# muzishen/IMAGDressing

Hardware: AMD Instinct MI355X
Metric: 512x512 50-step images/sec (whole node) (higher is better)
Workload: dtype bf16

## Files before the change

imagdressing_amd/_lib.py:

```python
from __future__ import annotations

import ctypes as C
import os

_HERE = os.path.dirname(os.path.abspath(__file__))
LIB_PATH = os.environ.get("IMD_LIB_PATH") or os.path.join(_HERE, "libimagdressing_hip.so")

ABI_VERSION = 9

u16p = C.POINTER(C.c_uint16)
f32p = C.POINTER(C.c_float)


class _Sized(C.Structure):

    def __init__(self, *args, **kw):
        super().__init__(*args, **kw)
        self.struct_bytes = C.sizeof(self)


class HeadsDest(C.Structure):
    _fields_ = [("ptr", C.c_void_p), ("kind", C.c_int), ("DP", C.c_int), ("L", C.c_int), ("scale", C.c_float)]


# ... 1 lines not shown
    _fields_ = [("struct_bytes", C.c_uint32), 
        ("x", C.c_void_p), ("w", C.c_void_p), ("out", C.c_void_p),
        ("M", C.c_int), ("N", C.c_int), ("K", C.c_int),
        ("Cin", C.c_int), ("taps", C.c_int), ("Hin", C.c_int), ("Win", C.c_int), ("Hout", C.c_int),
        ("Wout", C.c_int), ("stride", C.c_int), ("ups", C.c_int),
        ("x_pix_stride", C.c_int), ("out_ld", C.c_int), ("res_ld", C.c_int),
        ("bias", C.c_void_p), ("rowvec", C.c_void_p), ("rowvec_stride", C.c_int),
        ("res", C.c_void_p), ("out_scale", C.c_float), ("act", C.c_int), ("out_f32", C.c_int),
        ("mode", C.c_int), ("hC", C.c_int), ("hH", C.c_int), ("hD", C.c_int),
        ("hd", HeadsDest * 3), ("dtype", C.c_int), ("split_k", C.c_int), ("splitk_ws", C.c_void_p),
        ("x_bytes", C.c_uint32), ("w_bytes", C.c_uint32), ("flags", C.c_int),
        ("gn_a", C.c_void_p), ("gn_b", C.c_void_p), ("gn_silu", C.c_int), ("pad_br_only", C.c_int),
        ("splitk_counters", C.c_void_p),
        ("gn_stats_out", C.c_void_p), ("gn_stats_groups", C.c_int),
        ("gn_in_partial", C.c_void_p), ("gn_in_gamma", C.c_void_p), ("gn_in_beta", C.c_void_p),
        ("gn_in_nparts", C.c_int), ("gn_in_groups", C.c_int), ("gn_in_silu", C.c_int), ("gn_in_eps", C.c_float),
        ("gn_out_gamma", C.c_void_p), ("gn_out_beta", C.c_void_p), ("gn_out_eps", C.c_float), ("gn_out_silu", C.c_int), ("gn_out_groups", C.c_int), ("res_rows", C.c_int),
    ]


class FfParams(_Sized):
    _fields_ = [("struct_bytes", C.c_uint32), ("x", C.c_void_p), ("w1", C.c_void_p), ("b1", C.c_void_p), ("w2", C.c_void_p), ("b2", C.c_void_p), ("out", C.c_void_p),
                ("M", C.c_int), ("C", C.c_int), ("inner", C.c_int), ("x_ld", C.c_int), ("out_ld", C.c_int), ("ln", C.c_int),
                ("ln_eps", C.c_float), ("dtype", C.c_int)]


class AttnParams(_Sized):
    _fields_ = [("struct_bytes", C.c_uint32), 
        ("q", C.c_void_p), ("k1", C.c_void_p), ("v1t", C.c_void_p), ("k2", C.c_void_p), ("v2t", C.c_void_p),
        ("scale2", C.c_void_p), ("out", C.c_void_p),
        ("B", C.c_int), ("H", C.c_int), ("N", C.c_int), ("D", C.c_int),
        ("L1", C.c_int), ("L1P", C.c_int), ("kv1_bdiv", C.c_int),
        ("L2", C.c_int), ("L2P", C.c_int), ("kv2_bdiv", C.c_int),
        ("out_ld", C.c_int), ("dtype", C.c_int), ("flags", C.c_int), ("causal", C.c_int), ("k_pad_one", C.c_int),
        ("proj_w", C.c_void_p), ("proj_b", C.c_void_p), ("proj_res", C.c_void_p), ("proj_out", C.c_void_p),
        ("proj_res_ld", C.c_int), ("proj_out_ld", C.c_int), ("proj_counters", C.c_void_p),
        ("out_dup", C.c_void_p), ("phase2_out", C.c_void_p), ("phase2_rows", C.c_int),
    ]


class GroupNormParams(_Sized):
    _fields_ = [("struct_bytes", C.c_uint32), 
        ("x", C.c_void_p), ("y", C.c_void_p), ("gamma", C.c_void_p), ("beta", C.c_void_p), ("partial", C.c_void_p),
        ("B", C.c_int), ("HW", C.c_int), ("C", C.c_int), ("G", C.c_int), ("x_ld", C.c_int), ("y_ld", C.c_int),
        ("eps", C.c_float), ("silu", C.c_int), ("dtype", C.c_int), ("nparts", C.c_int),
    ]
# ... 28 lines not shown
    "imd_attention": (C.c_int, [C.POINTER(AttnParams), C.c_void_p]),
    "imd_attention_dup_supported": (C.c_int, [C.c_int, C.c_int, C.c_int]),
    "imd_attention_phase_split_supported": (C.c_int, [C.c_int]),
    "imd_attention_fp8": (C.c_int, [C.POINTER(AttnParams), C.c_int, C.c_int, C.c_int, C.c_void_p]),
    "imd_attn_quantize_fp8": (C.c_int, [C.c_void_p, C.c_void_p, C.c_int, C.c_long, C.c_int, C.c_int, C.c_float, C.c_int, C.c_void_p]),
    "imd_set_tuning": (C.c_int, [C.c_int, C.c_int]),
    "imd_get_tuning": (C.c_int, [C.c_int]),
    "imd_attn_padded_dims": (C.c_int, [C.c_int, C.POINTER(C.c_int), C.POINTER(C.c_int)]),
    "imd_groupnorm": (C.c_int, [C.POINTER(GroupNormParams), C.c_void_p]),
    "imd_groupnorm_coeffs": (C.c_int, [C.POINTER(GroupNormParams), C.c_void_p, C.c_void_p, C.c_void_p]),
    "imd_conv_patch_supported": (C.c_int, [C.POINTER(ConvGemmParams)]),
    "imd_conv_patch2_supported": (C.c_int, [C.POINTER(ConvGemmParams)]),
    "imd_conv_patch3_supported": (C.c_int, [C.POINTER(ConvGemmParams)]),
    "imd_conv_patch4_supported": (C.c_int, [C.POINTER(ConvGemmParams)]),
    "imd_conv_img_supported": (C.c_int, [C.POINTER(ConvGemmParams)]),
    "imd_conv_patch_stats_parts": (C.c_int, [C.POINTER(ConvGemmParams)]),
    "imd_conv_gemm_stats_parts": (C.c_int, [C.POINTER(ConvGemmParams), C.c_int]),
    "imd_conv_gemm_gn_out_supported": (C.c_int, [C.POINTER(ConvGemmParams)]),
    "imd_row_linear_gn_in_supported": (C.c_int, [C.POINTER(ConvGemmParams), C.c_int]),
    "imd_gemm_dma_supported": (C.c_int, [C.POINTER(ConvGemmParams)]),
    "imd_row_linear": (C.c_int, [C.POINTER(ConvGemmParams), C.c_int, C.c_float, C.c_void_p]),
    "imd_row_linear_supported": (C.c_int, [C.POINTER(ConvGemmParams)]),
    "imd_ff_geglu": (C.c_int, [C.POINTER(FfParams), C.c_void_p]),
    "imd_groupnorm_workspace_floats": (C.c_int, [C.c_int, C.c_int, C.c_int, C.c_int]),
    "imd_layernorm": (C.c_int, [C.POINTER(LayerNormParams), C.c_void_p]),
    "imd_softmax_rows": (C.c_int, [C.c_void_p, C.c_int, C.c_void_p, C.c_int, C.c_int, C.c_int, C.c_int, C.c_void_p]),
    "imd_ddim_cfg_step": (C.c_int, [C.POINTER(DdimParams), C.c_void_p]),
    "imd_ddim_cfg_step_rows": (C.c_int, [C.POINTER(DdimParams), C.c_void_p, C.c_void_p]),
    "imd_timestep_embedding": (C.c_int, [C.c_void_p, C.c_void_p, C.c_int, C.c_int, C.c_void_p]),
    "imd_add": (C.c_int, [C.c_void_p, C.c_int, C.c_void_p, C.c_int, C.c_void_p, C.c_int, C.c_long, C.c_int, C.c_float, C.c_int, C.c_void_p]),
    "imd_embed_tokens": (C.c_int, [C.c_void_p, C.c_int, C.c_void_p, C.c_int, C.c_void_p, C.c_void_p, C.c_long, C.c_int, C.c_int, C.c_void_p]),
    "imd_vit_assemble": (C.c_int, [C.c_void_p, C.c_void_p, C.c_void_p, C.c_void_p, C.c_int, C.c_int, C.c_int, C.c_int, C.c_void_p]),
    "imd_lincomb": (C.c_int, [C.POINTER(C.c_void_p), C.POINTER(C.c_float), C.c_int, C.c_void_p, C.c_long, C.c_void_p]),
    "imd_copy2d": (C.c_int, [C.c_void_p, C.c_int, C.c_void_p, C.c_int, C.c_long, C.c_int, C.c_void_p]),
    "imd_concat2": (C.c_int, [C.c_void_p, C.c_int, C.c_void_p, C.c_int, C.c_void_p, C.c_void_p, C.c_long, C.c_long, C.c_int, C.c_void_p]),
    "imd_concat2_gn_stats": (C.c_int, [C.c_void_p, C.c_int, C.c_void_p, C.c_int, C.c_void_p, C.c_void_p, C.c_int, C.c_int, C.c_int, C.c_int,
                                       C.c_void_p, C.c_int, C.c_void_p]),
    "imd_groupnorm_parts": (C.c_int, [C.c_int, C.c_int, C.c_int]),
    "imd_f32_to_16": (C.c_int, [C.c_void_p, C.c_void_p, C.c_long, C.c_int, C.c_void_p]),
}

_lib = None


class ImdError(RuntimeError):
    pass
# ... 23 lines not shown
```

imagdressing_amd/adapter/attention_processor.py:

```python
from __future__ import annotations

import math
from typing import Dict, Optional, Tuple

import torch
import torch.nn as nn

from .. import ops

bf16 = torch.bfloat16
LOG2E = math.log2(math.e)


class LoRALinearLayer(nn.Module):

    def __init__(self, in_features, out_features, rank=4, network_alpha=None):
        super().__init__()
        self.down = nn.Linear(in_features, rank, bias=False)
        self.up = nn.Linear(rank, out_features, bias=False)
        self.network_alpha = network_alpha
        self.rank = rank
        nn.init.normal_(self.down.weight, std=1 / rank)
        nn.init.zeros_(self.up.weight)

# ... 61 lines not shown
    if ent is None or ent[0] != key or not all(a is b for a, b in zip(ent[1], srcs)):
        t = torch.cat([t.detach().to(device=device, dtype=want) for t in srcs], 0).contiguous()
        ent = cache[which] = (key, tuple(srcs), t)
    return ent[2]


def _ln_folded_q(attn, gamma: torch.Tensor, beta: torch.Tensor, dtype, device, which: str = "q"):
    mods = [getattr(attn, n) for n in _W_PARTS[which]]
    srcs = tuple(m.weight for m in mods) + (gamma, beta)
    cache = attn.__dict__.setdefault("_imd_wcache", {})
    key = (_version_key(*srcs), dtype, str(device))
    ent = cache.get(which + "_ln")
    if ent is None or ent[0] != key or not all(a is b for a, b in zip(ent[1], srcs)):
        w = torch.cat([m.weight.detach().to(device=device, dtype=dtype) for m in mods], 0)
        ent = cache[which + "_ln"] = (key, srcs, ops.fold_layernorm_affine(w, None, gamma.to(device), beta.to(device)))
    return ent[2]


def _qkv_ln_ok(x: torch.Tensor) -> bool:
    return x.shape[-1] == 320 and x.shape[1] % 128 == 0 and ops.FUSED_LN


FUSED_LN_CHANNELS = (320, 640, 1280)


def _as_tokens(hidden_states: torch.Tensor, dtype):
    shape4 = None
    if hidden_states.dim() == 4:
        b, c, h, w = hidden_states.shape
        shape4 = (b, c, h, w)
        hidden_states = hidden_states.view(b, c, h * w).transpose(1, 2)
    if not hidden_states.is_cuda:
        from .._lib import ImdError
        raise ImdError("imagdressing_amd processors run on MI355X only: hidden_states is on " + str(hidden_states.device))
    return hidden_states.to(dtype).contiguous(), shape4


def _restore(out, shape4, like):
    if shape4 is not None:
        b, c, h, w = shape4
        out = out.transpose(-1, -2).reshape(b, c, h, w)
    return out


def _project_kv(tokens: torch.Tensor, wkv: torch.Tensor, heads: int):
    Bk, Lk, Kd = tokens.shape
# ... 93 lines not shown
        Be = ehs.shape[0]
        if B % Be:
            raise ValueError(f"encoder_hidden_states batch {Be} does not divide hidden_states batch {B}")
        return B // Be

    @staticmethod
    def _finish(attn, out, residual_given, like, shape4, ln_fused=False):
        if getattr(attn, "residual_connection", False) and not residual_given:
            if ln_fused:
                raise NotImplementedError("attn.residual_connection together with the engine's fused LayerNorm (imd_layernorm)")
            out = ops.add(out, _as_tokens(like, out.dtype)[0])
        if getattr(attn, "rescale_output_factor", 1.0) != 1.0:
            raise NotImplementedError("rescale_output_factor != 1 is not used by SD1.5")
        out = _restore(out, shape4, like)
        return out if out.dtype == like.dtype else out.to(like.dtype)


class AttnProcessor2_0(_FusedBase):

    fused_layernorm = True

    def __init__(self, cache_entries: int = 256):
        self._text = _TensorCache(capacity=cache_entries)

    def __call__(self, attn, hidden_states, encoder_hidden_states=None, attention_mask=None, temb=None, scale=1.0,
                 imd_residual=None, imd_layernorm=None, **kwargs):
        dt = _compute_dtype(attn, hidden_states, attention_mask)
        x, shape4 = _as_tokens(hidden_states, dt)
        dev = x.device
        wo, bo = _layer_weights(attn, "o", dt, dev), _layer_weights(attn, "bo", dt, dev)
        q_ln = None
        if imd_layernorm is not None:
            g, be, eps = imd_layernorm
            if encoder_hidden_states is not None and x.shape[-1] in FUSED_LN_CHANNELS:
                q_ln = _ln_folded_q(attn, g, be, dt, dev) + (eps,)
            elif encoder_hidden_states is None and _qkv_ln_ok(x):
                q_ln = _ln_folded_q(attn, g, be, dt, dev, "qkv") + (eps,)
            else:
                x = ops.layer_norm(x, g, be, eps)
        if encoder_hidden_states is None:
            out = _fused_attention(x, attn.heads, wq_or_qkv=_layer_weights(attn, "qkv", dt, dev), self_attn=True, wo=wo, bo=bo,
                                   residual=imd_residual, q_ln=q_ln)
        else:
            srcs = (encoder_hidden_states, attn.to_k.weight, attn.to_v.weight)
            kv = self._text.get(srcs, extra=(dt,))
            if kv is None:
                e = encoder_hidden_states.to(device=dev, dtype=dt).contiguous()
                kv = self._text.put(srcs, _project_kv(e, _layer_weights(attn, "kv", dt, dev), attn.heads), extra=(dt,))
            out = _fused_attention(x, attn.heads, wq_or_qkv=_layer_weights(attn, "q", dt, dev), self_attn=False, kv1=kv,
                                   kv1_bdiv=self._ehs_bdiv(x.shape[0], encoder_hidden_states), wo=wo, bo=bo,
                                   residual=imd_residual, q_ln=q_ln)
        return self._finish(attn, out, imd_residual is not None, hidden_states, shape4, ln_fused=imd_layernorm is not None)
# ... 339 lines not shown
```

imagdressing_amd/csrc/capi.cpp:

```cpp
#include <atomic>
#include <mutex>
#include <stdarg.h>
#include <stdio.h>
#include <string.h>

#include "imd_kernels.h"

namespace {
thread_local char g_err[512] = "";
}

int imd_set_error(const char* fmt, ...) {
    va_list ap;
    va_start(ap, fmt);
    vsnprintf(g_err, sizeof(g_err), fmt, ap);
    va_end(ap);
    return 1;
}

int imd_check_launch(const char* what) {
    hipError_t e = hipGetLastError();
    if (e != hipSuccess) return imd_set_error("%s: launch failed: %s", what, hipGetErrorString(e));
    return 0;
}
// ... 178 lines not shown
    if (p->mode == IMD_OUT_HEADS) {
        IMD_REQUIRE(p->hC > 0 && p->hH > 0 && p->hD > 0 && p->hC == p->hH * p->hD && p->N % p->hC == 0 && p->N / p->hC <= 3 && p->hD % 8 == 0,
                    "row_linear: bad head split C=%d H=%d D=%d", p->hC, p->hH, p->hD);
        IMD_REQUIRE(!p->out_f32, "row_linear: head-split output excludes fp32 output");
    }
    IMD_REQUIRE(!ln || ln_eps > 0.f, "row_linear: LayerNorm needs eps > 0");
    if (p->K == 320 && p->N == 960 && p->mode == IMD_OUT_HEADS) {
        IMD_REQUIRE(p->gn_in_partial == nullptr, "row_linear: the fused q / k / v projection has no GroupNorm prologue (gn_in_*)");
        return imd_launch_row_qkv(*p, ln, ln_eps, (hipStream_t)stream);
    }
    if (p->K == 640) return imd_launch_row_linear_k640(*p, ln, ln_eps, (hipStream_t)stream);
    if (p->K == 1280) return imd_launch_row_linear_k1280(*p, ln, ln_eps, (hipStream_t)stream);
    return imd_launch_row_linear(*p, ln, ln_eps, (hipStream_t)stream);
}

int imd_ff_geglu(const imd_ff_params* p, void* stream) {
    IMD_REQUIRE(p != nullptr, "ff_geglu: null params");
    IMD_REQUIRE_SIZE(p, "ff_geglu");
    IMD_REQUIRE(p->x && p->w1 && p->b1 && p->w2 && p->b2 && p->out, "ff_geglu: null pointer");
    IMD_REQUIRE(!p->ln || p->ln_eps > 0.f, "ff_geglu: LayerNorm needs eps > 0");
    return imd_launch_ff_geglu(*p, (hipStream_t)stream);
}

int imd_layernorm(const imd_layernorm_params* p, void* stream) {
    IMD_REQUIRE(p != nullptr, "layernorm: null params");
    IMD_REQUIRE_SIZE(p, "layernorm");
    IMD_REQUIRE(p->x && p->y && p->gamma && p->beta, "layernorm: null pointer");
    return imd_launch_layernorm(*p, (hipStream_t)stream);
}

int imd_embed_tokens(const uint16_t* table, int vocab, const uint16_t* pos, int T, const int64_t* ids, uint16_t* out, long rows, int C,
                     int dtype, void* stream) {
    IMD_REQUIRE(table && pos && ids && out, "embed_tokens: null pointer");
    return imd_launch_embed_tokens(table, vocab, pos, T, ids, out, rows, C, dtype, (hipStream_t)stream);
}

int imd_vit_assemble(const uint16_t* patches, const uint16_t* cls, const uint16_t* pos, uint16_t* out, int B, int P, int C, int dtype,
                     void* stream) {
    IMD_REQUIRE(patches && cls && pos && out, "vit_assemble: null pointer");
    return imd_launch_vit_assemble(patches, cls, pos, out, B, P, C, dtype, (hipStream_t)stream);
}

int imd_lincomb(const float* const* xs, const float* coefs, int n, float* out, long numel, void* stream) {
    IMD_REQUIRE(xs && coefs && out, "lincomb: null pointer");
    return imd_launch_lincomb(xs, coefs, n, out, numel, (hipStream_t)stream);
}
// ... 57 lines not shown
```

imagdressing_amd/csrc/imd_kernels.h:

```cpp
#pragma once
#include <hip/hip_runtime.h>
#include <stdint.h>

#include "../../include/imagdressing_hip.h"

typedef uint16_t bf16_t;
typedef imd_heads_dest HeadsDest;
typedef imd_conv_gemm_params ConvGemmParams;
typedef imd_attn_params AttnParams;
typedef imd_groupnorm_params GroupNormParams;
typedef imd_layernorm_params LayerNormParams;
typedef imd_ddim_params DdimParams;

enum { ACT_NONE = IMD_ACT_NONE, ACT_SILU = IMD_ACT_SILU, ACT_GEGLU = IMD_ACT_GEGLU, ACT_GELU = IMD_ACT_GELU, ACT_QUICK_GELU = IMD_ACT_QUICK_GELU };
enum { OUT_ROWMAJOR = IMD_OUT_ROWMAJOR, OUT_HEADS = IMD_OUT_HEADS };

int imd_set_error(const char* fmt, ...);
int imd_check_launch(const char* what);
int imd_lds_attr(const void* kern, int bytes, const char* what);
int imd_cu_count8();

int imd_conv_gemm_choose_cfg(int M, int N);
int imd_conv_gemm_choose_split(int M, int N, int K, int cfg);
int imd_launch_conv_gemm(const ConvGemmParams& p, int cfg, hipStream_t s);
// ... 9 lines not shown
bool imd_conv_patch64_supported(const ConvGemmParams& p);
int imd_launch_conv_patch64(const ConvGemmParams& p, hipStream_t s);
bool imd_conv_img_supported(const ConvGemmParams& p);
int imd_launch_conv_img(const ConvGemmParams& p, hipStream_t s);
int imd_conv_patch_stats_parts_of(const ConvGemmParams& p);
int imd_conv_gemm_stats_parts_of(const ConvGemmParams& p, int cfg);
bool imd_conv_gemm_gn_out_supported_of(const ConvGemmParams& p, int cfg);
bool imd_row_linear_gn_in_supported_of(const ConvGemmParams& p, int cfg);
int imd_launch_conv_patch(const ConvGemmParams& p, hipStream_t s);
bool imd_row_linear_supported(const ConvGemmParams& p);
int imd_launch_row_linear(const ConvGemmParams& p, int ln, float ln_eps, hipStream_t s);
bool imd_row_linear_k640_supported(const ConvGemmParams& p);
int imd_launch_row_linear_k640(const ConvGemmParams& p, int ln, float ln_eps, hipStream_t s);
bool imd_row_linear_k1280_supported(const ConvGemmParams& p);
int imd_launch_row_linear_k1280(const ConvGemmParams& p, int ln, float ln_eps, hipStream_t s);
bool imd_row_qkv_supported(const ConvGemmParams& p);
int imd_launch_row_qkv(const ConvGemmParams& p, int ln, float ln_eps, hipStream_t s);
bool imd_gemm_dma_supported(const ConvGemmParams& p);
int imd_launch_gemm_dma(const ConvGemmParams& p, hipStream_t s);
int imd_launch_gemm_dma128(const ConvGemmParams& p, int stages, hipStream_t s);
int imd_launch_gemm_dma256(const ConvGemmParams& p, int form, hipStream_t s);
bool imd_conv_dma_supported(const ConvGemmParams& p);
int imd_launch_ff_geglu(const imd_ff_params& p, hipStream_t s);
int imd_launch_attention(const AttnParams& p, hipStream_t s);
int imd_launch_attention_d40(const AttnParams& p, int variant, hipStream_t s);
int imd_launch_attention_fp8(const AttnParams& p, int eq, int ek, int ev, hipStream_t s);
int imd_launch_attn_quantize_fp8(const bf16_t* src, unsigned char* dst, int kind, long rows_or_groups, int LP, int exp2_scale,
                                 float pad_val, int dtype, hipStream_t s);
extern int g_attn_qw40;
extern int g_attn_xcd;
#ifdef IMD_ATTN_SWEEP
extern int g_attn_v80, g_attn_v160;
#endif
extern int g_gemm_flags;
int imd_attn_dpk(int D);
int imd_attn_dpv(int D);
int imd_launch_groupnorm(const GroupNormParams& p, hipStream_t s);
int imd_launch_groupnorm_coeffs(const GroupNormParams& p, float* ca, float* cb, hipStream_t s);
int imd_groupnorm_parts_of(int B, int HW, int C);
int imd_launch_concat2_gn_stats(const bf16_t* a, int Ca, const bf16_t* b, int Cb, const bf16_t* b_add, bf16_t* out, int B, int HW, int b_B, int G,
                                float* partial, int dtype, hipStream_t s);
int imd_launch_layernorm(const LayerNormParams& p, hipStream_t s);
int imd_launch_softmax_rows(const float* s_in, int s_ld, bf16_t* p_out, int p_ld, int rows, int cols, int dtype, hipStream_t s);
int imd_launch_ddim_cfg_step(const DdimParams& p, hipStream_t s);
int imd_launch_ddim_cfg_step_rows(const DdimParams& p, const float* guidance, hipStream_t s);
int imd_launch_timestep_embedding(const float* t, float* out, int B, int dim, hipStream_t s);
// ... 8 lines not shown
```

imagdressing_amd/ops.py:

```python
from __future__ import annotations

import functools
import ctypes as C
from typing import Dict, Optional, Sequence, Tuple

import torch

from . import _lib as L

ACT_NONE, ACT_SILU, ACT_GEGLU, ACT_GELU, ACT_QUICK_GELU = 0, 1, 2, 3, 4
bf16 = torch.bfloat16
f16 = torch.float16
DTYPE_CODE = {torch.bfloat16: 0, torch.float16: 1}


def _code(t: torch.Tensor, name: str = "tensor") -> int:
    try:
        return DTYPE_CODE[t.dtype]
    except KeyError:
        raise L.ImdError(f"{name}: expected a bfloat16 or float16 tensor, got {t.dtype}") from None


try:
    _raw_stream, _cur_dev = torch._C._cuda_getCurrentRawStream, torch._C._cuda_getDevice
# ... 94 lines not shown

def pad64(n: int) -> int:
    return (n + 63) // 64 * 64


PATCH_CONV = True
PATCH_MIN_W = 32
SPLITK_IN_KERNEL = False
FUSED_FF = True
FUSED_FF_MIN_ROWS = 24576
import os as _os
FUSED_GN_STATS = _os.environ.get("IMD_FUSED_GN_STATS", "1") != "0"
CFG_PAIR_DEDUP = _os.environ.get("IMD_CFG_PAIR_DEDUP", "1") != "0"
FUSED_GN_CONV = _os.environ.get("IMD_FUSED_GN_CONV", "0") == "1"
FUSED_GN_FINISH = _os.environ.get("IMD_FUSED_GN_FINISH", "0") == "1"
FUSED_GN_PROJ = _os.environ.get("IMD_FUSED_GN_PROJ", "1") != "0"
FUSED_CONCAT_STATS = _os.environ.get("IMD_FUSED_CONCAT_STATS", "1") != "0"
PERIODIC_RES = _os.environ.get("IMD_PERIODIC_RES", "1") != "0"
GENERIC_GN_STATS = _os.environ.get("IMD_GENERIC_GN_STATS", "0") == "1"
TEMB_TABLE = _os.environ.get("IMD_TEMB_TABLE", "1") != "0"
FUSED_GN_PROJ_CFGS = tuple(int(c) for c in _os.environ.get("IMD_FUSED_GN_PROJ_CFGS", "12,13,14").split(",") if c)
CFG_PAIR_ATTN = _os.environ.get("IMD_CFG_PAIR_ATTN", "1") != "0"
FUSED_LN = True
GEMM_TRACE = None
GEMM_EVENT_HOOK = None
_GEMM_TABLE = None
_CFG_DECISIONS: Dict[Tuple, Tuple[int, int]] = {}

TUNING_PER_CALL = 0x5A000000
ATTN_VARIANT_MAX = 13


import contextvars

_TUNING = contextvars.ContextVar("imd_tuning_scope", default=None)


class tuning_scope:

    def __init__(self, attn_variant=None, attn_xcd=None, gemm_flags=None):
        self.new = dict(attn_variant=attn_variant, attn_xcd=attn_xcd, gemm_flags=gemm_flags)

    def __enter__(self):
        merged = dict(_TUNING.get() or {})
        merged.update({k: v for k, v in self.new.items() if v is not None})
        self.token = _TUNING.set(merged if any(v is not None for v in merged.values()) else None)
# ... 283 lines not shown
    ks = torch.arange(16, device=dev)
    jk = torch.where(ks < 4, ks, torch.where(ks < 8, ks + 4, torch.where(ks < 12, ks - 4, ks)))
    cols = (16 * torch.arange(inner // 16, device=dev)[:, None] + jk[None, :]).reshape(inner // 32, 32)
    w2p = w2.float()[:, cols].permute(1, 0, 2).to(dtype).contiguous()
    return dict(w1=w1p, b1=b1p, w2=w2p, b2=b2.float().contiguous(), ln=gamma is not None, C=C, inner=inner)


def ff_geglu_fused(x2d: torch.Tensor, packed: dict, ln_eps: float = 1e-5, out: Optional[torch.Tensor] = None) -> torch.Tensor:
    ensure_device(x2d.device)
    M, C_ = x2d.shape
    dt = x2d.dtype
    if out is None:
        out = torch.empty((M, C_), dtype=dt, device=x2d.device)
    p = L.FfParams()
    p.x, p.w1, p.b1 = _dev(x2d, dt, "x"), _dev(packed["w1"], dt, "w1"), _dev(packed["b1"], torch.float32, "b1")
    p.w2, p.b2, p.out = _dev(packed["w2"], dt, "w2"), _dev(packed["b2"], torch.float32, "b2"), _dev(out, dt, "out")
    p.M, p.C, p.inner, p.x_ld, p.out_ld = M, packed["C"], packed["inner"], x2d.stride(0), out.stride(0)
    p.ln, p.ln_eps, p.dtype = int(packed["ln"]), float(ln_eps), _code(x2d, "x")
    _count("gemm_conv", 2.0 * M * packed["C"] * 2 * packed["inner"] + 2.0 * M * packed["inner"] * packed["C"])
    L.check(L.load().imd_ff_geglu(C.byref(p), _stream()))
    return out


def conv2d_nhwc(x: torch.Tensor, w: torch.Tensor, bias=None, *, taps=9, stride=1, ups=False, rowvec=None,
                rowvec_stride=0, rowvec_off=0, res=None, out_scale=1.0, act=ACT_NONE, out_f32=False, cfg=-1, split_k=0, gn=None,
                pad_br_only=False, gn_stats_groups=0, gn_out=None, gn_in=None) -> torch.Tensor:
    B, H, W, Cin = x.shape
    Cout = w.shape[0]
    Hl, Wl = (2 * H, 2 * W) if ups else (H, W)
    Ho, Wo = ((Hl + stride - 1) // stride, (Wl + stride - 1) // stride)
    M = B * Ho * Wo
    out = conv_gemm(x, w, M=M, N=Cout, Cin=Cin, taps=taps, Hin=H, Win=W, Hout=Ho, Wout=Wo, stride=stride, ups=ups,
                    bias=bias, rowvec=rowvec, rowvec_stride=rowvec_stride, rowvec_off=rowvec_off, res=res, out_scale=out_scale, act=act,
                    out_f32=out_f32, cfg=cfg, split_k=split_k, gn=gn, pad_br_only=pad_br_only, gn_stats_groups=gn_stats_groups, gn_out=gn_out, gn_in=gn_in)
    r = out.view(B, Ho, Wo, -1)
    if getattr(out, "_imd_gn_applied", False):
        r._imd_gn_applied = True
    st = getattr(out, "_imd_gn_stats", None)
    if st is not None:
        r._imd_gn_stats = st
    return r


ATTN_EVENT_HOOK = None


# ... 357 lines not shown
```

include/imagdressing_hip.h:

```cpp
#ifndef IMAGDRESSING_HIP_H
#define IMAGDRESSING_HIP_H

#include <stdint.h>

#ifdef __cplusplus
extern "C" {
#endif

#define IMD_ABI_VERSION 9

enum { IMD_ACT_NONE = 0, IMD_ACT_SILU = 1, IMD_ACT_GEGLU = 2, IMD_ACT_GELU = 3, IMD_ACT_QUICK_GELU = 4  };
enum { IMD_OUT_ROWMAJOR = 0, IMD_OUT_HEADS = 1 };
enum { IMD_DTYPE_BF16 = 0, IMD_DTYPE_F16 = 1 };

typedef struct imd_heads_dest {
    uint16_t* ptr;
    int kind;
    int DP;
    int L;
    float scale;
} imd_heads_dest;

#define IMD_TUNING_PER_CALL 0x5A000000
#define IMD_TUNING_TAG_MASK 0xFF000000u
// ... 66 lines not shown
    uint16_t* proj_out;
    int proj_res_ld, proj_out_ld;
    int* proj_counters;
    uint16_t* out_dup;
    float* phase2_out;
    int phase2_rows;
} imd_attn_params;

typedef struct imd_ff_params {
    uint32_t struct_bytes;
    const uint16_t* x;
    const uint16_t* w1;
    const float* b1;
    const uint16_t* w2;
    const float* b2;
    uint16_t* out;
    int M, C, inner;
    int x_ld, out_ld;
    int ln;
    float ln_eps;
    int dtype;
} imd_ff_params;

typedef struct imd_groupnorm_params {
    uint32_t struct_bytes;
    const uint16_t* x; uint16_t* y; const float* gamma; const float* beta;
    float* partial;
    int B, HW, C, G, x_ld, y_ld;
    float eps;
    int silu;
    int dtype;
    int nparts;
} imd_groupnorm_params;

typedef struct imd_layernorm_params {
    uint32_t struct_bytes;
    const uint16_t* x; uint16_t* y; const float* gamma; const float* beta;
    int rows, C, x_ld, y_ld;
    float eps;
    int dtype;
} imd_layernorm_params;

typedef struct imd_ddim_params {
    uint32_t struct_bytes;
    float* z;
    const float* eps;
// ... 26 lines not shown
int imd_conv_gemm_gn_out_supported(const imd_conv_gemm_params* p);
int imd_attention_dup_supported(int H, int N, int D);
int imd_attention_phase_split_supported(int D);
int imd_attn_padded_dims(int D, int* dpk, int* dpv);
int imd_set_tuning(int knob, int value);
int imd_get_tuning(int knob);

int imd_groupnorm(const imd_groupnorm_params* p, void* stream);
int imd_groupnorm_workspace_floats(int B, int HW, int C, int G);
int imd_groupnorm_coeffs(const imd_groupnorm_params* p, float* coef_a, float* coef_b, void* stream);
int imd_conv_patch_supported(const imd_conv_gemm_params* p);
int imd_conv_patch2_supported(const imd_conv_gemm_params* p);
int imd_conv_patch3_supported(const imd_conv_gemm_params* p);
int imd_conv_patch4_supported(const imd_conv_gemm_params* p);
int imd_conv_img_supported(const imd_conv_gemm_params* p);
int imd_conv_patch_stats_parts(const imd_conv_gemm_params* p);
int imd_conv_gemm_stats_parts(const imd_conv_gemm_params* p, int cfg);
int imd_gemm_dma_supported(const imd_conv_gemm_params* p);

int imd_row_linear(const imd_conv_gemm_params* p, int ln, float ln_eps, void* stream);
int imd_row_linear_supported(const imd_conv_gemm_params* p);

int imd_ff_geglu(const imd_ff_params* p, void* stream);

int imd_layernorm(const imd_layernorm_params* p, void* stream);
int imd_softmax_rows(const float* s, int s_ld, uint16_t* p, int p_ld, int rows, int cols, int dtype, void* stream);

int imd_ddim_cfg_step(const imd_ddim_params* p, void* stream);
int imd_ddim_cfg_step_rows(const imd_ddim_params* p, const float* guidance, void* stream);

int imd_timestep_embedding(const float* t, float* out, int B, int dim, void* stream);

int imd_add(const uint16_t* a, int a_ld, const uint16_t* b, int b_ld, uint16_t* out, int out_ld, long rows, int C, float b_scale, int dtype, void* stream);
int imd_embed_tokens(const uint16_t* table, int vocab, const uint16_t* pos, int T, const int64_t* ids, uint16_t* out, long rows, int C,
                     int dtype, void* stream);
int imd_vit_assemble(const uint16_t* patches, const uint16_t* cls, const uint16_t* pos, uint16_t* out, int B, int P, int C, int dtype,
                     void* stream);
int imd_lincomb(const float* const* xs, const float* coefs, int n, float* out, long numel, void* stream);
int imd_copy2d(const uint16_t* a, int a_ld, uint16_t* out, int out_ld, long rows, int C, void* stream);
int imd_concat2(const uint16_t* a, int Ca, const uint16_t* b, int Cb, const uint16_t* b_add, uint16_t* out, long rows, long b_rows, int dtype, void* stream);
int imd_concat2_gn_stats(const uint16_t* a, int Ca, const uint16_t* b, int Cb, const uint16_t* b_add, uint16_t* out, int B, int HW, int b_B, int G,
                         float* partial, int dtype, void* stream);
int imd_groupnorm_parts(int B, int HW, int C);
int imd_f32_to_16(const float* a, uint16_t* out, long n, int dtype, void* stream);

#ifdef __cplusplus
// ... 4 lines not shown
```

Before: 6.887.

## Fuse LayerNorm, text cross-attention and output projection into one kernel for C=320

Adds a single HIP kernel for the 320-channel text cross-attention layers. It applies LayerNorm, computes logits against precomputed (K·Wq)-folded matrices, runs softmax, and applies the precomputed (V·Wo) matrix plus bias and residual. Folding the projections into per-text-set packed operands (cached on the host side) removes the separate Q projection, the attention kernel and the output projection along with their intermediate round trips through memory. The trade-offs are a larger K dimension of 320 per head in place of 40, bf16 rounding of the folded weights, and a kernel fixed to C=320, 8 heads and at most 80 keys.

```diff
diff --git a/imagdressing_amd/_lib.py b/imagdressing_amd/_lib.py
--- a/imagdressing_amd/_lib.py
+++ b/imagdressing_amd/_lib.py
@@ -47,6 +47,12 @@
 class FfParams(_Sized):
     _fields_ = [("struct_bytes", C.c_uint32), ("x", C.c_void_p), ("w1", C.c_void_p), ("b1", C.c_void_p), ("w2", C.c_void_p), ("b2", C.c_void_p), ("out", C.c_void_p),
                 ("M", C.c_int), ("C", C.c_int), ("inner", C.c_int), ("x_ld", C.c_int), ("out_ld", C.c_int), ("ln", C.c_int),
+                ("ln_eps", C.c_float), ("dtype", C.c_int)]
+
+
+class XattnParams(_Sized):
+    _fields_ = [("struct_bytes", C.c_uint32), ("x", C.c_void_p), ("a", C.c_void_p), ("s0", C.c_void_p), ("b", C.c_void_p), ("bo", C.c_void_p), ("out", C.c_void_p),
+                ("M", C.c_int), ("C", C.c_int), ("heads", C.c_int), ("sets", C.c_int), ("rows_per_set", C.c_int), ("x_ld", C.c_int), ("out_ld", C.c_int),
                 ("ln_eps", C.c_float), ("dtype", C.c_int)]
 
 
@@ -121,6 +127,7 @@
     "imd_row_linear": (C.c_int, [C.POINTER(ConvGemmParams), C.c_int, C.c_float, C.c_void_p]),
     "imd_row_linear_supported": (C.c_int, [C.POINTER(ConvGemmParams)]),
     "imd_ff_geglu": (C.c_int, [C.POINTER(FfParams), C.c_void_p]),
+    "imd_text_xattn": (C.c_int, [C.POINTER(XattnParams), C.c_void_p]),
     "imd_groupnorm_workspace_floats": (C.c_int, [C.c_int, C.c_int, C.c_int, C.c_int]),
     "imd_layernorm": (C.c_int, [C.POINTER(LayerNormParams), C.c_void_p]),
     "imd_softmax_rows": (C.c_int, [C.c_void_p, C.c_int, C.c_void_p, C.c_int, C.c_int, C.c_int, C.c_int, C.c_void_p]),
diff --git a/imagdressing_amd/adapter/attention_processor.py b/imagdressing_amd/adapter/attention_processor.py
--- a/imagdressing_amd/adapter/attention_processor.py
+++ b/imagdressing_amd/adapter/attention_processor.py
@@ -107,6 +107,20 @@
 
 
 FUSED_LN_CHANNELS = (320, 640, 1280)
+
+
+def _text_xattn_ok(attn, x: torch.Tensor, ehs: torch.Tensor, residual, imd_layernorm) -> bool:
+    if imd_layernorm is None or residual is None or not (ops.FUSED_LN and ops.FUSED_TEXT_XATTN) or ops.ATTN_FP8:
+        return False
+    if x.dim() != 3 or ehs.dim() != 3 or x.shape[-1] != ops.XATTN_C or attn.heads != ops.XATTN_HEADS or ehs.shape[1] > ops.XATTN_KEYS:
+        return False
+    if residual is not x and not (residual.data_ptr() == x.data_ptr() and residual.shape == x.shape and residual.dtype == x.dtype
+                                  and residual.stride() == x.stride()):
+        return False
+    if any(getattr(getattr(attn, n), "bias", None) is not None for n in ("to_q", "to_k", "to_v")):
+        return False
+    B, N, _ = x.shape
+    return N % 128 == 0 and B * N >= ops.FUSED_TEXT_XATTN_MIN_ROWS and ehs.shape[0] >= 1 and B % ehs.shape[0] == 0
 
 
 def _as_tokens(hidden_states: torch.Tensor, dtype):
@@ -246,12 +260,32 @@
 
     def __init__(self, cache_entries: int = 256):
         self._text = _TensorCache(capacity=cache_entries)
+        self._xattn = _TensorCache(capacity=cache_entries)
+
+    def _text_xattn(self, attn, x, encoder_hidden_states, imd_layernorm, dt):
+        g, be, eps = imd_layernorm
+        dev = x.device
+        ob = attn.to_out[0].bias
+        srcs = (encoder_hidden_states, attn.to_q.weight, attn.to_k.weight, attn.to_v.weight, attn.to_out[0].weight, g, be) + (() if ob is None else (ob,))
+        packed = self._xattn.get(srcs, extra=(dt,))
+        if packed is None:
+            Cc = x.shape[-1]
+            wkv = _layer_weights(attn, "kv", dt, dev)
+            e = encoder_hidden_states.detach().to(device=dev, dtype=dt)
+            packed = self._xattn.put(srcs, ops.pack_text_xattn(e, _layer_weights(attn, "q", dt, dev), wkv[:Cc], wkv[Cc:], _layer_weights(attn, "o", dt, dev),
+                                                               _layer_weights(attn, "bo", dt, dev), g, be, heads=attn.heads, dtype=dt), extra=(dt,))
+        B, N, Cc = x.shape
+        bdiv = self._ehs_bdiv(B, encoder_hidden_states)
+        return ops.text_xattn_fused(x.view(B * N, Cc), packed, [i // bdiv for i in range(B)], eps).view(B, N, Cc)
 
     def __call__(self, attn, hidden_states, encoder_hidden_states=None, attention_mask=None, temb=None, scale=1.0,
                  imd_residual=None, imd_layernorm=None, **kwargs):
         dt = _compute_dtype(attn, hidden_states, attention_mask)
         x, shape4 = _as_tokens(hidden_states, dt)
         dev = x.device
+        if encoder_hidden_states is not None and _text_xattn_ok(attn, x, encoder_hidden_states, imd_residual, imd_layernorm):
+            out = self._text_xattn(attn, x, encoder_hidden_states, imd_layernorm, dt)
+            return self._finish(attn, out, True, hidden_states, shape4, ln_fused=True)
         wo, bo = _layer_weights(attn, "o", dt, dev), _layer_weights(attn, "bo", dt, dev)
         q_ln = None
         if imd_layernorm is not None:
diff --git a/imagdressing_amd/csrc/capi.cpp b/imagdressing_amd/csrc/capi.cpp
--- a/imagdressing_amd/csrc/capi.cpp
+++ b/imagdressing_amd/csrc/capi.cpp
@@ -224,6 +224,14 @@
     return imd_launch_ff_geglu(*p, (hipStream_t)stream);
 }
 
+int imd_text_xattn(const imd_xattn_params* p, void* stream) {
+    IMD_REQUIRE(p != nullptr, "text_xattn: null params");
+    IMD_REQUIRE_SIZE(p, "text_xattn");
+    IMD_REQUIRE(p->x && p->a && p->s0 && p->b && p->bo && p->out, "text_xattn: null pointer");
+    IMD_REQUIRE(p->ln_eps > 0.f, "text_xattn: LayerNorm needs eps > 0");
+    return imd_launch_text_xattn(*p, (hipStream_t)stream);
+}
+
 int imd_layernorm(const imd_layernorm_params* p, void* stream) {
     IMD_REQUIRE(p != nullptr, "layernorm: null params");
     IMD_REQUIRE_SIZE(p, "layernorm");
diff --git a/imagdressing_amd/csrc/imd_kernels.h b/imagdressing_amd/csrc/imd_kernels.h
--- a/imagdressing_amd/csrc/imd_kernels.h
+++ b/imagdressing_amd/csrc/imd_kernels.h
@@ -55,6 +55,7 @@
 int imd_launch_gemm_dma256(const ConvGemmParams& p, int form, hipStream_t s);
 bool imd_conv_dma_supported(const ConvGemmParams& p);
 int imd_launch_ff_geglu(const imd_ff_params& p, hipStream_t s);
+int imd_launch_text_xattn(const imd_xattn_params& p, hipStream_t s);
 int imd_launch_attention(const AttnParams& p, hipStream_t s);
 int imd_launch_attention_d40(const AttnParams& p, int variant, hipStream_t s);
 int imd_launch_attention_fp8(const AttnParams& p, int eq, int ek, int ev, hipStream_t s);
diff --git a/imagdressing_amd/csrc/xattn_fused.hip b/imagdressing_amd/csrc/xattn_fused.hip
--- /dev/null
+++ b/imagdressing_amd/csrc/xattn_fused.hip
@@ -0,0 +1,273 @@
+#include <type_traits>
+#include "gemm_common.h"
+#include "lds_dma.h"
+
+namespace {
+
+constexpr int XA_C = 320, XA_H = 8, XA_KP = 96;
+constexpr int XA_T1 = 24;
+constexpr int XA_SLAB = 20480;
+constexpr int XA_OFF_B = 2 * XA_SLAB;
+constexpr int XA_OFF_DUMP = 4 * XA_SLAB;
+constexpr int XA_OFF_P = XA_OFF_DUMP + 1024;
+constexpr int XA_OFF_S0 = XA_OFF_P + 8 * 5 * 1024;
+constexpr int XA_OFF_BO = XA_OFF_S0 + XA_H * XA_KP * 4;
+constexpr int XA_LDS = XA_OFF_BO + XA_C * 4;
+
+template <bool F16>
+__global__ __launch_bounds__(512, 1) void text_xattn320_kernel(const imd_xattn_params p) {
+    using E = El<F16>;
+    extern __shared__ __attribute__((aligned(16))) char smem[];
+    const int tid = threadIdx.x;
+    const int lane = tid & 63;
+    const int wave = __builtin_amdgcn_readfirstlane(tid >> 6);
+    const int hi = lane >> 5, col = lane & 31;
+    const int rb = wave & 3, hh = wave >> 2;
+    const int m0 = blockIdx.x * 128;
+    const int m = m0 + rb * 32 + col;
+    const int set = m0 / p.rows_per_set;
+
+    const uint32_t x_bytes = (uint32_t)(((size_t)(p.M - 1) * p.x_ld + XA_C) * 2);
+    const __amdgpu_buffer_rsrc_t rs_x = __builtin_amdgcn_make_buffer_rsrc(const_cast<uint16_t*>(p.x), 0, x_bytes, 0x00020000);
+    const uint32_t xoff = (uint32_t)m * (uint32_t)(p.x_ld * 2) + hi * 16;
+    uint4 xf[20];
+#pragma unroll
+    for (int s = 0; s < 20; ++s) xf[s] = buf_load16(rs_x, m < p.M ? xoff + s * 32 : OOB);
+    const float* s0g = p.s0 + (size_t)set * (XA_H * XA_KP);
+    const float s0a = s0g[tid], s0b = tid < XA_H * XA_KP - 512 ? s0g[tid + 512] : 0.f;
+    const float bov = tid < XA_C ? p.bo[tid] : 0.f;
+
+    const v4i_t ds_a = raw_rsrc(p.a + (size_t)set * (XA_T1 * XA_SLAB / 2), (uint32_t)(XA_T1 * XA_SLAB));
+    const v4i_t ds_b = raw_rsrc(p.b + (size_t)set * (XA_T1 * XA_SLAB / 2), (uint32_t)(XA_T1 * XA_SLAB));
+    uint32_t aoff[3], boff[3];
+#pragma unroll
+    for (int j = 0; j < 3; ++j) {
+        const int id = j * 8 + wave;
+        const int q = id * 64 + lane;
+        const int ra = q / 20, pa = q - ra * 20;
+        aoff[j] = id < 20 ? (uint32_t)(ra * 320 + ((pa ^ ((ra >> 2) & 3)) << 4)) : OOB;
+        const int rw = q >> 2, pw = q & 3;
+        boff[j] = id < 20 ? (uint32_t)(rw * 64 + ((pw ^ ((rw >> 2) & 3)) << 4)) : OOB;
+    }
+    const uint32_t lds0 = (uint32_t)(uintptr_t)smem;
+    auto stage = [&](const v4i_t& rsrc, const uint32_t* off, uint32_t ring, int slot, int slab) {
+#pragma unroll
+        for (int j = 0; j < 3; ++j) {
+            const int id = j * 8 + wave;
+            const uint32_t dst = id < 20 ? lds0 + ring + (uint32_t)(slot * XA_SLAB) + (uint32_t)id * 1024u : lds0 + XA_OFF_DUMP;
+            dma16(rsrc, dst, off[j] == OOB ? OOB : off[j] + (uint32_t)slab * XA_SLAB);
+        }
+    };
+    stage(ds_a, aoff, 0, 0, 0); stage(ds_a, aoff, XA_OFF_B, 0, 1);
+#pragma unroll
+    for (int s = 0; s < 20; ++s) asm volatile("" : "+v"(xf[s].x), "+v"(xf[s].y), "+v"(xf[s].z), "+v"(xf[s].w));
+    {
+        float* s0s = reinterpret_cast<float*>(smem + XA_OFF_S0);
+        s0s[tid] = s0a;
+        if (tid < XA_H * XA_KP - 512) s0s[tid + 512] = s0b;
+        if (tid < XA_C) reinterpret_cast<float*>(smem + XA_OFF_BO)[tid] = bov;
+    }
+
+    {
+        float sum = 0.f;
+#pragma unroll
+        for (int s = 0; s < 20; ++s) {
+            float f[8];
+            unpack8<F16>(xf[s], f);
+#pragma unroll
+            for (int e = 0; e < 8; ++e) sum += f[e];
+        }
+        sum += __shfl_xor(sum, 32);
+        const float mean = sum * (1.0f / XA_C);
+        float sq = 0.f;
+#pragma unroll
+        for (int s = 0; s < 20; ++s) asm volatile("" : "+v"(xf[s].x), "+v"(xf[s].y), "+v"(xf[s].z), "+v"(xf[s].w));
+#pragma unroll
+        for (int s = 0; s < 20; ++s) {
+            float f[8];
+            unpack8<F16>(xf[s], f);
+#pragma unroll
+            for (int e = 0; e < 8; ++e) { const float d = f[e] - mean; sq = fmaf(d, d, sq); }
+        }
+        sq += __shfl_xor(sq, 32);
+        const float rstd = rsqrtf(sq * (1.0f / XA_C) + p.ln_eps);
+        const float shift = -mean * rstd;
+#pragma unroll
+        for (int s = 0; s < 20; ++s) asm volatile("" : "+v"(xf[s].x), "+v"(xf[s].y), "+v"(xf[s].z), "+v"(xf[s].w));
+#pragma unroll
+        for (int s = 0; s < 20; ++s) {
+            float f[8];
+            unpack8<F16>(xf[s], f);
+#pragma unroll
+            for (int e = 0; e < 8; ++e) f[e] = fmaf(f[e], rstd, shift);
+            xf[s] = pack8<F16>(f);
+        }
+    }
+
+    f32x16 acc_out[5], S[3];
+#pragma unroll
+    for (int cb = 0; cb < 5; ++cb)
+#pragma unroll
+        for (int r = 0; r < 16; ++r) acc_out[cb][r] = 0.f;
+#pragma unroll
+    for (int kb = 0; kb < 3; ++kb)
+#pragma unroll
+        for (int r = 0; r < 16; ++r) S[kb][r] = 0.f;
+
+    const uint32_t sw = (uint32_t)((col >> 2) & 3);
+    const uint32_t p_even = (((uint32_t)hi) ^ sw) << 4, p_odd = (((uint32_t)(2 + hi)) ^ sw) << 4;
+    const int arow = (hh * 32 + col) * 320;
+    const int brow = (hh * 160 + col) * 64;
+    uint4* px = reinterpret_cast<uint4*>(smem + XA_OFF_P);
+    const float* s0s = reinterpret_cast<const float*>(smem + XA_OFF_S0);
+
+    auto gemm1 = [&](int hp, auto kbc, auto khc, int at) {
+        constexpr int kb = decltype(kbc)::value, kh = decltype(khc)::value;
+        if (kh == 0) {
+            const float* sb = s0s + (hh * 4 + hp) * XA_KP + kb * 32 + 4 * hi;
+#pragma unroll
+            for (int q = 0; q < 4; ++q) {
+                const float4 b = *reinterpret_cast<const float4*>(sb + 8 * q);
+                S[kb][4 * q] = b.x; S[kb][4 * q + 1] = b.y; S[kb][4 * q + 2] = b.z; S[kb][4 * q + 3] = b.w;
+            }
+        }
+        const char* As = smem + at + arow;
+#pragma unroll
+        for (int sl = 0; sl < 10; ++sl) {
+            const uint4 af = *reinterpret_cast<const uint4*>(As + (sl >> 1) * 64 + ((sl & 1) ? p_odd : p_even));
+            S[kb] = E::mfma(af, xf[kh * 10 + sl], S[kb]);
+        }
+    };
+    auto gemm2 = [&](auto hsc, auto kbc, int at) {
+        constexpr int hs = decltype(hsc)::value, kb2 = decltype(kbc)::value;
+        const char* Bs = smem + at + brow;
+#pragma unroll
+        for (int ks = 0; ks < (kb2 == 2 ? 1 : 2); ++ks) {
+            const uint4 pf = px[((hs * 4 + rb) * 5 + kb2 * 2 + ks) * 64 + lane];
+#pragma unroll
+            for (int cb = 0; cb < 5; ++cb) {
+                const uint4 bf = *reinterpret_cast<const uint4*>(Bs + cb * 2048 + (ks ? p_odd : p_even));
+                acc_out[cb] = E::mfma(bf, pf, acc_out[cb]);
+            }
+        }
+    };
+    auto softmax_publish = [&]() {
+        __syncthreads();
+        float mx = S[0][0];
+#pragma unroll
+        for (int k = 0; k < 3; ++k)
+#pragma unroll
+            for (int r = 0; r < 16; ++r) mx = fmaxf(mx, S[k][r]);
+        mx = fmaxf(mx, __shfl_xor(mx, 32));
+        float sum = 0.f;
+#pragma unroll
+        for (int k = 0; k < 3; ++k)
+#pragma unroll
+            for (int r = 0; r < 16; ++r) { S[k][r] = __builtin_amdgcn_exp2f(S[k][r] - mx); sum += S[k][r]; }
+        sum += __shfl_xor(sum, 32);
+        const float inv = 1.0f / sum;
+#pragma unroll
+        for (int f = 0; f < 5; ++f) {
+            float v[8];
+#pragma unroll
+            for (int e = 0; e < 8; ++e) v[e] = S[f >> 1][8 * (f & 1) + e] * inv;
+            px[(wave * 5 + f) * 64 + lane] = pack8<F16>(v);
+        }
+    };
+    auto open_step = [&]() {
+        dma_wait();
+        __syncthreads();
+    };
+    using I0 = std::integral_constant<int, 0>; using I1 = std::integral_constant<int, 1>; using I2 = std::integral_constant<int, 2>;
+
+    auto fill = [&](auto fc) {
+        constexpr int f = decltype(fc)::value, slot = f & 1, nslot = slot ^ 1;
+        open_step();
+        if (f < 2) { stage(ds_a, aoff, 0, nslot, 2 * f + 2); stage(ds_a, aoff, XA_OFF_B, nslot, 2 * f + 3); }
+        else { stage(ds_a, aoff, 0, nslot, 6); stage(ds_b, boff, XA_OFF_B, nslot, 0); }
+        gemm1(0, fc, I0{}, slot * XA_SLAB);
+        __builtin_amdgcn_sched_barrier(0);
+        gemm1(0, fc, I1{}, XA_OFF_B + slot * XA_SLAB);
+        if (f == 2) softmax_publish();
+    };
+    fill(I0{}); fill(I1{}); fill(I2{});
+
+    auto steady = [&](int hp, auto uc) {
+        constexpr int u = decltype(uc)::value, slot = (u + 1) & 1, nslot = slot ^ 1;
+        const int t = 6 * hp + u;
+        open_step();
+        if (t + 1 < XA_T1) { stage(ds_a, aoff, 0, nslot, t + 1); stage(ds_b, boff, XA_OFF_B, nslot, t - 5); }
+        else { stage(ds_b, boff, XA_OFF_B, nslot, 18); stage(ds_b, boff, 0, nslot, 19); }
+        gemm1(hp, std::integral_constant<int, (u >> 1)>{}, std::integral_constant<int, (u & 1)>{}, slot * XA_SLAB);
+        gemm2(std::integral_constant<int, u / 3>{}, std::integral_constant<int, u % 3>{}, XA_OFF_B + slot * XA_SLAB);
+        if (u == 5) softmax_publish();
+    };
+#pragma unroll 1
+    for (int hp = 1; hp < 4; ++hp) {
+        steady(hp, I0{}); steady(hp, I1{}); steady(hp, I2{});
+        steady(hp, std::integral_constant<int, 3>{}); steady(hp, std::integral_constant<int, 4>{}); steady(hp, std::integral_constant<int, 5>{});
+    }
+
+    auto drain = [&](auto dc) {
+        constexpr int d = decltype(dc)::value, slot = (d + 1) & 1, nslot = slot ^ 1;
+        constexpr int u0 = 2 * d, u1 = 2 * d + 1;
+        open_step();
+        if (d < 2) { stage(ds_b, boff, XA_OFF_B, nslot, 20 + 2 * d); stage(ds_b, boff, 0, nslot, 21 + 2 * d); }
+        gemm2(std::integral_constant<int, u0 / 3>{}, std::integral_constant<int, u0 % 3>{}, XA_OFF_B + slot * XA_SLAB);
+        __builtin_amdgcn_sched_barrier(0);
+        gemm2(std::integral_constant<int, u1 / 3>{}, std::integral_constant<int, u1 % 3>{}, slot * XA_SLAB);
+    };
+    drain(I0{}); drain(I1{}); drain(I2{});
+
+    const float* bos = reinterpret_cast<const float*>(smem + XA_OFF_BO);
+    const uint32_t o_bytes = (uint32_t)(((size_t)(p.M - 1) * p.out_ld + XA_C) * 2);
+    const __amdgpu_buffer_rsrc_t rs_o = __builtin_amdgcn_make_buffer_rsrc(p.out, 0, o_bytes, 0x00020000);
+    const uint32_t rbase = (uint32_t)m * (uint32_t)(p.x_ld * 2), obase = (uint32_t)m * (uint32_t)(p.out_ld * 2);
+    uint2 res[5][4];
+#pragma unroll
+    for (int cb = 0; cb < 5; ++cb)
+#pragma unroll
+        for (int q = 0; q < 4; ++q) {
+            const int n = hh * 160 + cb * 32 + 8 * q + 4 * hi;
+            res[cb][q] = buf_load8(rs_x, m < p.M ? rbase + (uint32_t)(n * 2) : OOB);
+        }
+#pragma unroll
+    for (int cb = 0; cb < 5; ++cb)
+#pragma unroll
+        for (int t = 0; t < 2; ++t) {
+            uint32_t pk[2][2];
+#pragma unroll
+            for (int qq = 0; qq < 2; ++qq) {
+                const int q = 2 * t + qq, n = hh * 160 + cb * 32 + 8 * q + 4 * hi;
+                const float4 bb = *reinterpret_cast<const float4*>(bos + n);
+                const float v0 = acc_out[cb][4 * q] + bb.x + E::lo(res[cb][q].x), v1 = acc_out[cb][4 * q + 1] + bb.y + E::hi(res[cb][q].x);
+                const float v2 = acc_out[cb][4 * q + 2] + bb.z + E::lo(res[cb][q].y), v3 = acc_out[cb][4 * q + 3] + bb.w + E::hi(res[cb][q].y);
+                pk[qq][0] = E::pack2(v0, v1); pk[qq][1] = E::pack2(v2, v3);
+            }
+            const auto r0 = __builtin_amdgcn_permlane32_swap(pk[0][0], pk[1][0], false, false);
+            const auto r1 = __builtin_amdgcn_permlane32_swap(pk[0][1], pk[1][1], false, false);
+            typedef __attribute__((__vector_size__(4 * sizeof(uint32_t)))) uint32_t v4u_t;
+            const v4u_t w = {r0[0], r1[0], r0[1], r1[1]};
+            const int n8 = hh * 160 + cb * 32 + 16 * t + 8 * hi;
+            __builtin_amdgcn_raw_buffer_store_b128(w, rs_o, (int)(m < p.M ? obase + (uint32_t)(n8 * 2) : OOB), 0, 0);
+        }
+}
+
+}
+
+int imd_launch_text_xattn(const imd_xattn_params& p, hipStream_t s) {
+    if (p.C != XA_C || p.heads != XA_H) return imd_set_error("text_xattn: built for C = 320, 8 heads (got %d, %d)", p.C, p.heads);
+    if (p.M <= 0 || (p.x_ld % 8) || (p.out_ld % 8) || p.x_ld < XA_C || p.out_ld < XA_C) return imd_set_error("text_xattn: bad geometry M=%d x_ld=%d out_ld=%d", p.M, p.x_ld, p.out_ld);
+    if (p.sets <= 0 || p.rows_per_set <= 0 || (p.rows_per_set % 128) || (size_t)p.sets * p.rows_per_set < (size_t)p.M)
+        return imd_set_error("text_xattn: rows_per_set=%d must be a multiple of 128 and sets=%d must cover M=%d rows", p.rows_per_set, p.sets, p.M);
+    if (((size_t)(p.M - 1) * p.x_ld + XA_C) * 2 >= 0xffffffffull || ((size_t)(p.M - 1) * p.out_ld + XA_C) * 2 >= 0xffffffffull)
+        return imd_set_error("text_xattn: operand larger than 4 GiB");
+    if (p.dtype != IMD_DTYPE_BF16 && p.dtype != IMD_DTYPE_F16) return imd_set_error("text_xattn: unknown dtype %d", p.dtype);
+    const bool h = p.dtype == IMD_DTYPE_F16;
+    const void* kern = h ? reinterpret_cast<const void*>(text_xattn320_kernel<true>) : reinterpret_cast<const void*>(text_xattn320_kernel<false>);
+    if (int rc_attr = imd_lds_attr(kern, XA_LDS, "text_xattn")) return rc_attr;
+    const dim3 grid((unsigned)((p.M + 127) / 128));
+    if (h) hipLaunchKernelGGL(text_xattn320_kernel<true>, grid, dim3(512), XA_LDS, s, p);
+    else hipLaunchKernelGGL(text_xattn320_kernel<false>, grid, dim3(512), XA_LDS, s, p);
+    return imd_check_launch("text_xattn");
+}
diff --git a/imagdressing_amd/ops.py b/imagdressing_amd/ops.py
--- a/imagdressing_amd/ops.py
+++ b/imagdressing_amd/ops.py
@@ -140,6 +140,8 @@
 FUSED_GN_PROJ_CFGS = tuple(int(c) for c in _os.environ.get("IMD_FUSED_GN_PROJ_CFGS", "12,13,14").split(",") if c)
 CFG_PAIR_ATTN = _os.environ.get("IMD_CFG_PAIR_ATTN", "1") != "0"
 FUSED_LN = True
+FUSED_TEXT_XATTN = _os.environ.get("IMD_FUSED_TEXT_XATTN", "1") != "0"
+FUSED_TEXT_XATTN_MIN_ROWS = 16384
 GEMM_TRACE = None
 GEMM_EVENT_HOOK = None
 _GEMM_TABLE = None
@@ -469,6 +471,73 @@
     return out
 
 
+XATTN_C, XATTN_HEADS, XATTN_KEYS, XATTN_KEYS_PAD = 320, 8, 80, 96
+XATTN_PAD_LOGIT = -1.0e30
+_XATTN_SLOT_KEY = (0, 1, 2, 3, 8, 9, 10, 11, 4, 5, 6, 7, 12, 13, 14, 15)
+
+
+def pack_text_xattn(text: torch.Tensor, wq: torch.Tensor, wk: torch.Tensor, wv: torch.Tensor, wo: torch.Tensor, bo: Optional[torch.Tensor],
+                    gamma: torch.Tensor, beta: torch.Tensor, heads: int = XATTN_HEADS, dtype=None, bq: Optional[torch.Tensor] = None) -> dict:
+    dtype = dtype or wq.dtype
+    Cc = wq.shape[0]
+    sets, Lk, _ = text.shape
+    if Cc != XATTN_C or heads != XATTN_HEADS or Lk > XATTN_KEYS:
+        raise L.ImdError(f"pack_text_xattn: built for C = 320, 8 heads, <= 80 keys (got C={Cc}, heads={heads}, keys={Lk})")
+    D = Cc // heads
+    dev = wq.device
+    qs = D ** -0.5 * 1.4426950408889634
+    tf = text.detach().to(device=dev, dtype=torch.float32)
+    wqf, wkf, wvf, wof = (t.detach().float() for t in (wq, wk, wv, wo))
+    gf, bf = gamma.detach().to(device=dev, dtype=torch.float32), beta.detach().to(device=dev, dtype=torch.float32)
+    K = (tf @ wkf.t()).view(sets, Lk, heads, D).permute(0, 2, 1, 3)
+    V = (tf @ wvf.t()).view(sets, Lk, heads, D).permute(0, 2, 1, 3)
+    wqh = (wqf * gf[None, :]).view(heads, D, Cc)
+    qb = wqf @ bf
+    if bq is not None:
+        qb = qb + bq.detach().to(device=dev, dtype=torch.float32)
+    KP = XATTN_KEYS_PAD
+    A = torch.zeros(sets, heads, KP, Cc, dtype=torch.float32, device=dev)
+    A[:, :, :Lk] = qs * torch.einsum("shld,hdc->shlc", K, wqh)
+    s0 = torch.full((sets, heads, KP), XATTN_PAD_LOGIT, dtype=torch.float32, device=dev)
+    s0[:, :, :Lk] = qs * torch.einsum("shld,hd->shl", K, qb.view(heads, D))
+    Bm = torch.zeros(sets, heads, KP, Cc, dtype=torch.float32, device=dev)
+    Bm[:, :, :Lk] = torch.einsum("shld,chd->shlc", V, wof.view(Cc, heads, D))
+    a = A.view(sets, 2, 4, 3, 32, 2, Cc // 2).permute(0, 2, 3, 5, 1, 4, 6).reshape(sets, 24, 64, Cc // 2).to(dtype).contiguous()
+    slot = torch.tensor(_XATTN_SLOT_KEY, device=dev)
+    order = (16 * torch.arange(KP // 16, device=dev)[:, None] + slot[None, :]).reshape(-1)
+    b = Bm[:, :, order].view(sets, 2, 4, 3, 32, Cc).permute(0, 2, 1, 3, 5, 4).reshape(sets, 24, Cc, 32).to(dtype).contiguous()
+    bov = torch.zeros(Cc, dtype=torch.float32, device=dev) if bo is None else bo.detach().to(device=dev, dtype=torch.float32).contiguous()
+    return dict(a=a, s0=s0.contiguous(), b=b, bo=bov, sets=sets, keys=Lk, C=Cc, heads=heads)
+
+
+def text_xattn_fused(x2d: torch.Tensor, packed: dict, text_set_of_image, ln_eps: float = 1e-5, out: Optional[torch.Tensor] = None) -> torch.Tensor:
+    ensure_device(x2d.device)
+    M, C_ = x2d.shape
+    dt = x2d.dtype
+    sets_of = tuple(int(s) for s in text_set_of_image)
+    images = len(sets_of)
+    if images == 0 or M % images or (M // images) % 128:
+        raise L.ImdError(f"text_xattn_fused: {M} rows are not {images} images of a multiple of 128 tokens")
+    group = sets_of.count(0)
+    if group == 0 or images % group or any(s != i // group for i, s in enumerate(sets_of)) or sets_of[-1] >= packed["sets"]:
+        raise L.ImdError(f"text_xattn_fused: text sets {sets_of} are not contiguous groups of equal size over {packed['sets']} packed sets")
+    ns = packed["sets"]
+    if C_ != XATTN_C or tuple(packed["a"].shape) != (ns, 24, 64, XATTN_C // 2) or tuple(packed["b"].shape) != (ns, 24, XATTN_C, 32) \
+            or tuple(packed["s0"].shape) != (ns, XATTN_HEADS, XATTN_KEYS_PAD) or packed["bo"].numel() != XATTN_C:
+        raise L.ImdError("text_xattn_fused: operands are not what pack_text_xattn builds (the kernel streams them by fixed offsets)")
+    if out is None:
+        out = torch.empty((M, C_), dtype=dt, device=x2d.device)
+    p = L.XattnParams()
+    p.x, p.a, p.s0 = _dev(x2d, dt, "x"), _dev(packed["a"], dt, "a"), _dev(packed["s0"], torch.float32, "s0")
+    p.b, p.bo, p.out = _dev(packed["b"], dt, "b"), _dev(packed["bo"], torch.float32, "bo"), _dev(out, dt, "out")
+    p.M, p.C, p.heads, p.sets, p.rows_per_set = M, packed["C"], packed["heads"], packed["sets"], (M // images) * group
+    p.x_ld, p.out_ld, p.ln_eps, p.dtype = x2d.stride(0), out.stride(0), float(ln_eps), _code(x2d, "x")
+    _count("gemm_conv", 2.0 * M * C_ * C_ * 2)
+    _count("attention", 4.0 * M * C_ * packed["keys"])
+    L.check(L.load().imd_text_xattn(C.byref(p), _stream()))
+    return out
+
+
 def conv2d_nhwc(x: torch.Tensor, w: torch.Tensor, bias=None, *, taps=9, stride=1, ups=False, rowvec=None,
                 rowvec_stride=0, rowvec_off=0, res=None, out_scale=1.0, act=ACT_NONE, out_f32=False, cfg=-1, split_k=0, gn=None,
                 pad_br_only=False, gn_stats_groups=0, gn_out=None, gn_in=None) -> torch.Tensor:
diff --git a/include/imagdressing_hip.h b/include/imagdressing_hip.h
--- a/include/imagdressing_hip.h
+++ b/include/imagdressing_hip.h
@@ -112,6 +112,21 @@
     int dtype;
 } imd_ff_params;
 
+typedef struct imd_xattn_params {
+    uint32_t struct_bytes;
+    const uint16_t* x;
+    const uint16_t* a;
+    const float* s0;
+    const uint16_t* b;
+    const float* bo;
+    uint16_t* out;
+    int M, C, heads, sets;
+    int rows_per_set;
+    int x_ld, out_ld;
+    float ln_eps;
+    int dtype;
+} imd_xattn_params;
+
 typedef struct imd_groupnorm_params {
     uint32_t struct_bytes;
     const uint16_t* x; uint16_t* y; const float* gamma; const float* beta;
@@ -184,6 +199,8 @@
 int imd_row_linear_supported(const imd_conv_gemm_params* p);
 
 int imd_ff_geglu(const imd_ff_params* p, void* stream);
+
+int imd_text_xattn(const imd_xattn_params* p, void* stream);
 
 int imd_layernorm(const imd_layernorm_params* p, void* stream);
 int imd_softmax_rows(const float* s, int s_ld, uint16_t* p, int p_ld, int rows, int cols, int dtype, void* stream);
```

After: 6.928, median of 6. No clear change (+0.6%).
